# NYXFLOWER/TIP

Measured on AMD Instinct MI355X. Metric: D-D edges aggregated/sec (encoder fwd+bwd), higher is better.
Workload: dtype f32; 1 GPU; TIP-cat full encoder, BioSNAP (645 drugs, 19081 proteins, R=1097), 1xMI355X config; mod=cat, directed_dd_edges=8326508, relations=1097, parallelism=single GPU, launch=hipGraph replay of the captured step, rccl_ranks=0

## Files before the change

tip_amd/csrc/tipk_slab_xb.hip:

```cpp
#include <stdlib.h>
#include "tipk_common.h"

namespace {

struct SxArgs {
    const float* in; int64_t n_slabs, slab_stride; int n_rows;
    const float* row_scale; const float* addend; int relu;
    float* x;
    const float* basis; const float* root; int n_bases, d_out;
    float* xb;
    float* xroot;
};

__global__ __launch_bounds__(1024) void sum_slabs_xb_kernel(SxArgs a) {
    __shared__ float red[1024];
    __shared__ float xs[64];
    constexpr int lanes = 16, epb = 64;
    const int t = threadIdx.x, e = t % epb, j = t / epb;
    const int64_t count = (int64_t)a.n_rows * 32;
    const int64_t i = (int64_t)blockIdx.x * epb + e;
    float s = 0.f;
    if (i < count) {
        const float* p = a.in + i;
        int64_t k = j;
        for (; k + 3 * lanes < a.n_slabs; k += 4 * lanes) {
            const float v0 = p[k * a.slab_stride], v1 = p[(k + lanes) * a.slab_stride];
            const float v2 = p[(k + 2 * lanes) * a.slab_stride], v3 = p[(k + 3 * lanes) * a.slab_stride];
            s += v0; s += v1; s += v2; s += v3;
        }
        for (; k < a.n_slabs; k += lanes) s += p[k * a.slab_stride];
    }
    red[t] = s;
    __syncthreads();
    if (j == 0) {
        float v = 0.f;
        if (i < count) {
            v = red[e];
            for (int q = 1; q < lanes; ++q) v += red[q * epb + e];
            if (a.row_scale) v *= a.row_scale[i / 32];
            if (a.addend) v += a.addend[i];
            if (a.relu) v = fmaxf(v, 0.f);
            a.x[i] = v;
        }
        xs[e] = v;
    }
    __syncthreads();
    const int row0 = (int)blockIdx.x * 2;
    const int n_xb = a.n_bases * a.d_out, n_cols = n_xb + a.d_out;
    for (int n = t; n < n_cols; n += 1024) {
        const bool is_root = n >= n_xb;
        const int b = is_root ? 0 : n / a.d_out, c = is_root ? n - n_xb : n - b * a.d_out;
        const float* w = is_root ? a.root + c : a.basis + (int64_t)b * 32 * a.d_out + c;
        float wv[32];
#pragma unroll
        for (int k = 0; k < 32; ++k) wv[k] = w[k * a.d_out];
        float acc0 = 0.f, acc1 = 0.f;
#pragma unroll
        for (int k = 0; k < 32; ++k) { acc0 = fmaf(xs[k], wv[k], acc0); acc1 = fmaf(xs[32 + k], wv[k], acc1); }
        if (is_root) {
            a.xroot[(int64_t)row0 * a.d_out + c] = acc0;
            if (row0 + 1 < a.n_rows) a.xroot[(int64_t)(row0 + 1) * a.d_out + c] = acc1;
        } else {
            a.xb[((int64_t)row0 * a.n_bases + b) * 32 + c] = acc0;
            if (row0 + 1 < a.n_rows) a.xb[((int64_t)(row0 + 1) * a.n_bases + b) * 32 + c] = acc1;
        }
    }
}

}

extern "C" int tipk_sum_slabs_xb(const float* slabs, int64_t n_slabs, int64_t slab_stride, int64_t n_rows, int d_in,
                                 const float* row_scale, const float* addend, int relu, float* x,
                                 const float* basis, const float* root, int n_bases, int d_out, float* xb, float* xroot,
                                 tipk_stream_t stream) {
    if (d_in != 32 || d_out < 1 || d_out > 32 || n_bases < 1) return TIPK_EUNSUPPORTED;
    if (!slabs || !x || !basis || !root || !xb || !xroot || n_slabs < 1 || n_rows < 1 || slab_stride < n_rows * 32) return TIPK_EINVAL;
    const int64_t blocks = tipk_ceil_div(n_rows, 2);
    if (blocks > 0x7fffffffLL) return TIPK_EUNSUPPORTED;
    SxArgs a;
    a.in = slabs; a.n_slabs = n_slabs; a.slab_stride = slab_stride; a.n_rows = (int)n_rows;
    a.row_scale = row_scale; a.addend = addend; a.relu = relu; a.x = x;
    a.basis = basis; a.root = root; a.n_bases = n_bases; a.d_out = d_out; a.xb = xb; a.xroot = xroot;
    hipLaunchKernelGGL(sum_slabs_xb_kernel, dim3((unsigned)blocks), dim3(1024), 0, (hipStream_t)stream, a);
    TIPK_RETURN_LAUNCH();
}
```

tip_amd/csrc/tipk_slabs.h:

```cpp
#pragma once
#include "tipk_common.h"

namespace {

struct SlabArgs {
    const float* in; int64_t n_slabs, slab_stride, count; float alpha; int accumulate;
    const float* row_scale; int64_t cols; const float* addend; int relu; const float* gate; float* out;
    int lanes;
};
constexpr int SLAB_VEC4 = 1, SLAB_VEC16 = 2;
constexpr int SLAB_RED_FLOATS = 4096;

__device__ __forceinline__ void slab_sum_body(const SlabArgs& a, int block, float* red) {
    const int first = 0;
    const float* __restrict__ in = a.in;
    if (a.lanes == SLAB_VEC16) {
        const int e4 = threadIdx.x & 63, j = threadIdx.x >> 6;
        const int64_t i = (int64_t)(block - first) * 256 + e4 * 4;
        float4 s = make_float4(0.f, 0.f, 0.f, 0.f);
        if (i < a.count) {
            const float4* p = reinterpret_cast<const float4*>(in + i);
            const int64_t st4 = a.slab_stride / 4;
            int64_t k = j;
            for (; k + 48 < a.n_slabs; k += 64) {
                const float4 v0 = p[k * st4], v1 = p[(k + 16) * st4], v2 = p[(k + 32) * st4], v3 = p[(k + 48) * st4];
                s.x += v0.x; s.y += v0.y; s.z += v0.z; s.w += v0.w;
                s.x += v1.x; s.y += v1.y; s.z += v1.z; s.w += v1.w;
                s.x += v2.x; s.y += v2.y; s.z += v2.z; s.w += v2.w;
                s.x += v3.x; s.y += v3.y; s.z += v3.z; s.w += v3.w;
            }
            if (k < a.n_slabs) {
                float4 v[3];
#pragma unroll
                for (int u = 0; u < 3; ++u) v[u] = p[(k + 16 * u < a.n_slabs ? k + 16 * u : k) * st4];
#pragma unroll
                for (int u = 0; u < 3; ++u)
                    if (k + 16 * u < a.n_slabs) { s.x += v[u].x; s.y += v[u].y; s.z += v[u].z; s.w += v[u].w; }
            }
        }
        *reinterpret_cast<float4*>(red + j * 256 + e4 * 4) = s;
        __syncthreads();
        const int e = threadIdx.x;
        const int64_t o = (int64_t)(block - first) * 256 + e;
        if (e < 256 && o < a.count) {
            float t = red[e];
#pragma unroll
            for (int q = 1; q < 16; ++q) t += red[q * 256 + e];
            t *= a.alpha;
            if (a.row_scale) t *= a.row_scale[o / a.cols];
            if (a.addend) t += a.addend[o];
            if (a.accumulate) t += a.out[o];
            if (a.relu) t = fmaxf(t, 0.f);
            if (a.gate && !(a.gate[o] > 0.f)) t = 0.f;
            a.out[o] = t;
        }
        return;
    }
    if (a.lanes == SLAB_VEC4) {
        const int64_t i = ((int64_t)(block - first) * 1024 + threadIdx.x) * 4;
        if (i >= a.count) return;
        const float4* p = reinterpret_cast<const float4*>(in + i);
        const int64_t st4 = a.slab_stride / 4;
        float4 s[4];
#pragma unroll
        for (int j = 0; j < 4; ++j) s[j] = make_float4(0.f, 0.f, 0.f, 0.f);
        int64_t k = 0;
        for (; k + 8 <= a.n_slabs; k += 8) {
            float4 v[8];
#pragma unroll
            for (int u = 0; u < 8; ++u) v[u] = p[(k + u) * st4];
#pragma unroll
            for (int u = 0; u < 8; ++u) { s[u & 3].x += v[u].x; s[u & 3].y += v[u].y; s[u & 3].z += v[u].z; s[u & 3].w += v[u].w; }
        }
        {
            float4 v[8];
#pragma unroll
            for (int u = 0; u < 8; ++u) {
                const int64_t kc = k + u < a.n_slabs ? k + u : (a.n_slabs > 0 ? a.n_slabs - 1 : 0);
                v[u] = a.n_slabs > 0 ? p[kc * st4] : make_float4(0.f, 0.f, 0.f, 0.f);
            }
#pragma unroll
            for (int u = 0; u < 8; ++u)
                if (k + u < a.n_slabs) { s[u & 3].x += v[u].x; s[u & 3].y += v[u].y; s[u & 3].z += v[u].z; s[u & 3].w += v[u].w; }
        }
        float r[4] = {((s[0].x + s[1].x) + s[2].x) + s[3].x, ((s[0].y + s[1].y) + s[2].y) + s[3].y,
                      ((s[0].z + s[1].z) + s[2].z) + s[3].z, ((s[0].w + s[1].w) + s[2].w) + s[3].w};
        const float rs = a.row_scale ? a.row_scale[i / a.cols] : 1.f;
        float4 ad = make_float4(0.f, 0.f, 0.f, 0.f), ac = ad, gt = make_float4(1.f, 1.f, 1.f, 1.f);
        if (a.addend) ad = *reinterpret_cast<const float4*>(a.addend + i);
        if (a.accumulate) ac = *reinterpret_cast<const float4*>(a.out + i);
        if (a.gate) gt = *reinterpret_cast<const float4*>(a.gate + i);
        const float adv[4] = {ad.x, ad.y, ad.z, ad.w}, acv[4] = {ac.x, ac.y, ac.z, ac.w}, gtv[4] = {gt.x, gt.y, gt.z, gt.w};
#pragma unroll
        for (int c = 0; c < 4; ++c) {
            float t = r[c] * a.alpha;
            if (a.row_scale) t *= rs;
            if (a.addend) t += adv[c];
            if (a.accumulate) t += acv[c];
            if (a.relu) t = fmaxf(t, 0.f);
            if (a.gate && !(gtv[c] > 0.f)) t = 0.f;
            r[c] = t;
        }
        *reinterpret_cast<float4*>(a.out + i) = make_float4(r[0], r[1], r[2], r[3]);
        return;
    }
    const int lanes = a.lanes, epb = 1024 / lanes;
    const int e = threadIdx.x % epb, j = threadIdx.x / epb;
    const int64_t i = (int64_t)(block - first) * epb + e;
    float s = 0.f;
    if (i < a.count) {
        const float* p = in + i;
        int64_t k = j;
        for (; k + 3 * lanes < a.n_slabs; k += 4 * lanes) {
            const float v0 = p[k * a.slab_stride], v1 = p[(k + lanes) * a.slab_stride];
            const float v2 = p[(k + 2 * lanes) * a.slab_stride], v3 = p[(k + 3 * lanes) * a.slab_stride];
            s += v0; s += v1; s += v2; s += v3;
        }
        for (; k < a.n_slabs; k += lanes) s += p[k * a.slab_stride];
    }
    red[threadIdx.x] = s;
    __syncthreads();
    if (j == 0 && i < a.count) {
        s = red[e];
        for (int q = 1; q < lanes; ++q) s += red[q * epb + e];
        s *= a.alpha;
        if (a.row_scale) s *= a.row_scale[i / a.cols];
        if (a.addend) s += a.addend[i];
        if (a.accumulate) s += a.out[i];
        if (a.relu) s = fmaxf(s, 0.f);
        if (a.gate && !(a.gate[i] > 0.f)) s = 0.f;
        a.out[i] = s;
    }
}

inline int64_t fill_slab_args(const tipk_slab_sum_desc& d, SlabArgs& a, int* rc) {
    *rc = TIPK_OK;
    if (d.n_slabs < 0 || d.count < 0 || (d.row_scale && d.cols <= 0)) { *rc = TIPK_EINVAL; return 0; }
    if (d.count == 0) return 0;
    if (!d.out || (d.n_slabs > 0 && !d.in)) { *rc = TIPK_EINVAL; return 0; }
    a.in = d.in; a.n_slabs = d.n_slabs; a.slab_stride = d.slab_stride; a.count = d.count; a.alpha = d.alpha;
    a.accumulate = d.accumulate; a.row_scale = d.row_scale; a.cols = d.cols; a.addend = d.addend; a.relu = d.relu;
    a.gate = d.gate; a.out = d.out;
    a.lanes = (d.n_slabs >= 32 && tipk_ceil_div(d.count, 64) < 2048) ? 16 : 4;
    const auto al16 = [](const void* q) { return (reinterpret_cast<uintptr_t>(q) & 15) == 0; };
    const bool vec = d.count % 4 == 0 && d.slab_stride % 4 == 0 && al16(d.in) && al16(d.out) && al16(d.addend) && al16(d.gate) &&
                     (!d.row_scale || d.cols % 4 == 0);
    if (a.lanes == 4 && vec && d.count >= 4096) a.lanes = SLAB_VEC4;
    else if (a.lanes == 16 && vec) a.lanes = SLAB_VEC16;
    if (a.lanes == SLAB_VEC4) return tipk_ceil_div(d.count, 4096);
    if (a.lanes == SLAB_VEC16) return tipk_ceil_div(d.count, 256);
    return tipk_ceil_div(d.count, 1024 / a.lanes);
}

}
```

Before: 42.75 billion edges/s.

## Process eight rows per block in fused slab-sum and basis projection kernel

The fused slab-sum plus basis/root projection kernel now handles 8 rows per block on a float4-vectorized path instead of 2 rows with scalar loads. Each thread's 32 weights are reused across 8 rows, and the weight loads are issued while the slab loads are still in flight. Slab loads for small slab counts are batched, and epilogue operands are fetched early. The cost is more registers and fewer blocks, which may lower occupancy, plus extra template and debug paths.

```diff
diff --git a/tip_amd/csrc/tipk_slab_xb.hip b/tip_amd/csrc/tipk_slab_xb.hip
--- a/tip_amd/csrc/tipk_slab_xb.hip
+++ b/tip_amd/csrc/tipk_slab_xb.hip
@@ -1,68 +1,63 @@
 #include <stdlib.h>
 #include "tipk_common.h"
+#include "tipk_slabs.h"
 
 namespace {
 
 struct SxArgs {
-    const float* in; int64_t n_slabs, slab_stride; int n_rows;
-    const float* row_scale; const float* addend; int relu;
-    float* x;
+    SlabArgs s;
+    int n_rows;
     const float* basis; const float* root; int n_bases, d_out;
     float* xb;
     float* xroot;
 };
 
+template <int ROWS, bool WEARLY>
 __global__ __launch_bounds__(1024) void sum_slabs_xb_kernel(SxArgs a) {
-    __shared__ float red[1024];
-    __shared__ float xs[64];
-    constexpr int lanes = 16, epb = 64;
-    const int t = threadIdx.x, e = t % epb, j = t / epb;
-    const int64_t count = (int64_t)a.n_rows * 32;
-    const int64_t i = (int64_t)blockIdx.x * epb + e;
-    float s = 0.f;
-    if (i < count) {
-        const float* p = a.in + i;
-        int64_t k = j;
-        for (; k + 3 * lanes < a.n_slabs; k += 4 * lanes) {
-            const float v0 = p[k * a.slab_stride], v1 = p[(k + lanes) * a.slab_stride];
-            const float v2 = p[(k + 2 * lanes) * a.slab_stride], v3 = p[(k + 3 * lanes) * a.slab_stride];
-            s += v0; s += v1; s += v2; s += v3;
-        }
-        for (; k < a.n_slabs; k += lanes) s += p[k * a.slab_stride];
-    }
-    red[t] = s;
-    __syncthreads();
-    if (j == 0) {
-        float v = 0.f;
-        if (i < count) {
-            v = red[e];
-            for (int q = 1; q < lanes; ++q) v += red[q * epb + e];
-            if (a.row_scale) v *= a.row_scale[i / 32];
-            if (a.addend) v += a.addend[i];
-            if (a.relu) v = fmaxf(v, 0.f);
-            a.x[i] = v;
-        }
-        xs[e] = v;
-    }
-    __syncthreads();
-    const int row0 = (int)blockIdx.x * 2;
+    __shared__ __attribute__((aligned(16))) float red[ROWS == 8 ? SLAB_RED_FLOATS : 1024];
+    __shared__ __attribute__((aligned(16))) float xs[ROWS * 32];
+    const int t = threadIdx.x;
     const int n_xb = a.n_bases * a.d_out, n_cols = n_xb + a.d_out;
-    for (int n = t; n < n_cols; n += 1024) {
+    float wv[32];
+    auto load_weights = [&](int n) __attribute__((always_inline)) {
         const bool is_root = n >= n_xb;
         const int b = is_root ? 0 : n / a.d_out, c = is_root ? n - n_xb : n - b * a.d_out;
         const float* w = is_root ? a.root + c : a.basis + (int64_t)b * 32 * a.d_out + c;
-        float wv[32];
 #pragma unroll
         for (int k = 0; k < 32; ++k) wv[k] = w[k * a.d_out];
-        float acc0 = 0.f, acc1 = 0.f;
+    };
+    SlabArgs s = a.s;
+    s.lanes = ROWS == 8 ? SLAB_VEC16 : 16;
+    slab_sum_body<true>(s, (int)blockIdx.x, red, xs, [&]() __attribute__((always_inline)) {
+        if (WEARLY && t < n_cols) load_weights(t);
+    });
+    __syncthreads();
+    const int row0 = (int)blockIdx.x * ROWS;
+    for (int n = t; n < n_cols; n += 1024) {
+        if (!WEARLY || n != t) load_weights(n);
+        asm volatile("" ::: "memory");
+        const bool is_root = n >= n_xb;
+        const int b = is_root ? 0 : n / a.d_out, c = is_root ? n - n_xb : n - b * a.d_out;
+        float acc[ROWS];
 #pragma unroll
-        for (int k = 0; k < 32; ++k) { acc0 = fmaf(xs[k], wv[k], acc0); acc1 = fmaf(xs[32 + k], wv[k], acc1); }
-        if (is_root) {
-            a.xroot[(int64_t)row0 * a.d_out + c] = acc0;
-            if (row0 + 1 < a.n_rows) a.xroot[(int64_t)(row0 + 1) * a.d_out + c] = acc1;
-        } else {
-            a.xb[((int64_t)row0 * a.n_bases + b) * 32 + c] = acc0;
-            if (row0 + 1 < a.n_rows) a.xb[((int64_t)(row0 + 1) * a.n_bases + b) * 32 + c] = acc1;
+        for (int r = 0; r < ROWS; ++r) acc[r] = 0.f;
+#pragma unroll
+        for (int k = 0; k < 32; k += 4) {
+            __builtin_amdgcn_sched_barrier(0);
+#pragma unroll
+            for (int r = 0; r < ROWS; ++r) {
+                const float4 xv = *reinterpret_cast<const float4*>(xs + r * 32 + k);
+                acc[r] = fmaf(xv.x, wv[k], acc[r]); acc[r] = fmaf(xv.y, wv[k + 1], acc[r]);
+                acc[r] = fmaf(xv.z, wv[k + 2], acc[r]); acc[r] = fmaf(xv.w, wv[k + 3], acc[r]);
+            }
+        }
+#pragma unroll
+        for (int r = 0; r < ROWS; ++r) asm volatile("" : "+v"(acc[r]));
+#pragma unroll
+        for (int r = 0; r < ROWS; ++r) {
+            if (row0 + r >= a.n_rows) break;
+            if (is_root) a.xroot[(int64_t)(row0 + r) * a.d_out + c] = acc[r];
+            else a.xb[((int64_t)(row0 + r) * a.n_bases + b) * 32 + c] = acc[r];
         }
     }
 }
@@ -75,12 +70,29 @@
                                  tipk_stream_t stream) {
     if (d_in != 32 || d_out < 1 || d_out > 32 || n_bases < 1) return TIPK_EUNSUPPORTED;
     if (!slabs || !x || !basis || !root || !xb || !xroot || n_slabs < 1 || n_rows < 1 || slab_stride < n_rows * 32) return TIPK_EINVAL;
-    const int64_t blocks = tipk_ceil_div(n_rows, 2);
-    if (blocks > 0x7fffffffLL) return TIPK_EUNSUPPORTED;
     SxArgs a;
-    a.in = slabs; a.n_slabs = n_slabs; a.slab_stride = slab_stride; a.n_rows = (int)n_rows;
-    a.row_scale = row_scale; a.addend = addend; a.relu = relu; a.x = x;
+    a.s.in = slabs; a.s.n_slabs = n_slabs; a.s.slab_stride = slab_stride; a.s.count = n_rows * 32; a.s.alpha = 1.f;
+    a.s.accumulate = 0; a.s.row_scale = row_scale; a.s.cols = 32; a.s.addend = addend; a.s.relu = relu; a.s.gate = nullptr;
+    a.s.out = x;
+    a.n_rows = (int)n_rows;
     a.basis = basis; a.root = root; a.n_bases = n_bases; a.d_out = d_out; a.xb = xb; a.xroot = xroot;
-    hipLaunchKernelGGL(sum_slabs_xb_kernel, dim3((unsigned)blocks), dim3(1024), 0, (hipStream_t)stream, a);
+    const int dbg = tipk_option(TIPK_OPT_DP_DEBUG);
+    (void)dbg;
+    const auto al16 = [](const void* q) { return (reinterpret_cast<uintptr_t>(q) & 15) == 0; };
+    const bool vec = slab_stride % 4 == 0 && al16(slabs) && al16(x) && al16(addend) && !TIPK_DBG(dbg & 4096);
+    a.s.lanes = vec ? SLAB_VEC16 : 16;
+    const int64_t blocks = tipk_ceil_div(n_rows, vec ? 8 : 2);
+    if (blocks > 0x7fffffffLL || n_rows > 0x7fffffffLL / 32) return TIPK_EUNSUPPORTED;
+    const dim3 grid((unsigned)blocks), block(1024);
+    hipStream_t st = (hipStream_t)stream;
+#ifdef TIPK_DEBUG
+    if (dbg & 8192) {
+        if (vec) hipLaunchKernelGGL((sum_slabs_xb_kernel<8, false>), grid, block, 0, st, a);
+        else hipLaunchKernelGGL((sum_slabs_xb_kernel<2, false>), grid, block, 0, st, a);
+        TIPK_RETURN_LAUNCH();
+    }
+#endif
+    if (vec) hipLaunchKernelGGL((sum_slabs_xb_kernel<8, true>), grid, block, 0, st, a);
+    else hipLaunchKernelGGL((sum_slabs_xb_kernel<2, true>), grid, block, 0, st, a);
     TIPK_RETURN_LAUNCH();
 }
diff --git a/tip_amd/csrc/tipk_slabs.h b/tip_amd/csrc/tipk_slabs.h
--- a/tip_amd/csrc/tipk_slabs.h
+++ b/tip_amd/csrc/tipk_slabs.h
@@ -11,9 +11,116 @@
 constexpr int SLAB_VEC4 = 1, SLAB_VEC16 = 2;
 constexpr int SLAB_RED_FLOATS = 4096;
 
-__device__ __forceinline__ void slab_sum_body(const SlabArgs& a, int block, float* red) {
+constexpr int SLAB_BATCH = 6;
+struct SlabNoHook { __device__ __forceinline__ void operator()() const {} };
+
+struct SlabEpilogue { float rs, ad, ac; bool open; };
+__device__ __forceinline__ SlabEpilogue slab_epilogue_loads(const SlabArgs& a, int64_t o, bool fin) {
+    SlabEpilogue q = {1.f, 0.f, 0.f, true};
+    if (fin) {
+        if (a.row_scale) q.rs = a.row_scale[o / a.cols];
+        if (a.addend) q.ad = a.addend[o];
+        if (a.accumulate) q.ac = a.out[o];
+        if (a.gate) q.open = a.gate[o] > 0.f;
+    }
+    return q;
+}
+__device__ __forceinline__ float slab_epilogue(const SlabArgs& a, float t, const SlabEpilogue& q) {
+    t = __fmul_rn(t, a.alpha);
+    if (a.row_scale) t = __fmul_rn(t, q.rs);
+    if (a.addend) t = __fadd_rn(t, q.ad);
+    if (a.accumulate) t = __fadd_rn(t, q.ac);
+    if (a.relu) t = fmaxf(t, 0.f);
+    if (a.gate && !q.open) t = 0.f;
+    return t;
+}
+
+template <bool CHAIN = false, class Hook = SlabNoHook>
+__device__ __forceinline__ void slab_sum_body(const SlabArgs& a, int block, float* red, float* keep = nullptr, Hook after_issue = Hook()) {
     const int first = 0;
     const float* __restrict__ in = a.in;
+    if (CHAIN && (a.lanes == SLAB_VEC16 || a.lanes == 16)) {
+        const bool vec = a.lanes == SLAB_VEC16;
+        const int epb = vec ? 256 : 64, e = threadIdx.x, j = threadIdx.x >> 6;
+        const int64_t o = (int64_t)block * epb + e;
+        const bool fin = e < epb && o < a.count;
+        const bool batch = a.n_slabs > 0 && a.n_slabs <= 16 * SLAB_BATCH;
+        SlabEpilogue q;
+        if (vec) {
+            const int e4 = threadIdx.x & 63;
+            const int64_t i = (int64_t)block * 256 + e4 * 4;
+            const bool live = i < a.count;
+            const float4* p = reinterpret_cast<const float4*>(in + (live ? i : 0));
+            const int64_t st4 = a.slab_stride / 4;
+            float4 s = make_float4(0.f, 0.f, 0.f, 0.f);
+            if (batch) {
+                float4 v[SLAB_BATCH];
+#pragma unroll
+                for (int u = 0; u < SLAB_BATCH; ++u) v[u] = p[(j + 16 * u < a.n_slabs ? j + 16 * u : 0) * st4];
+                q = slab_epilogue_loads(a, o, fin);
+                after_issue();
+#pragma unroll
+                for (int u = 0; u < SLAB_BATCH; ++u)
+                    if (live && j + 16 * u < a.n_slabs) { s.x += v[u].x; s.y += v[u].y; s.z += v[u].z; s.w += v[u].w; }
+            } else {
+                q = slab_epilogue_loads(a, o, fin);
+                after_issue();
+                if (live) {
+                    int64_t k = j;
+                    for (; k + 48 < a.n_slabs; k += 64) {
+                        const float4 v0 = p[k * st4], v1 = p[(k + 16) * st4], v2 = p[(k + 32) * st4], v3 = p[(k + 48) * st4];
+                        s.x += v0.x; s.y += v0.y; s.z += v0.z; s.w += v0.w;
+                        s.x += v1.x; s.y += v1.y; s.z += v1.z; s.w += v1.w;
+                        s.x += v2.x; s.y += v2.y; s.z += v2.z; s.w += v2.w;
+                        s.x += v3.x; s.y += v3.y; s.z += v3.z; s.w += v3.w;
+                    }
+                    for (; k < a.n_slabs; k += 16) { const float4 v0 = p[k * st4]; s.x += v0.x; s.y += v0.y; s.z += v0.z; s.w += v0.w; }
+                }
+            }
+            *reinterpret_cast<float4*>(red + j * 256 + e4 * 4) = s;
+        } else {
+            const int64_t i = (int64_t)block * 64 + (threadIdx.x & 63);
+            const bool live = i < a.count;
+            const float* p = in + (live ? i : 0);
+            float s = 0.f;
+            if (batch) {
+                float v[SLAB_BATCH];
+#pragma unroll
+                for (int u = 0; u < SLAB_BATCH; ++u) v[u] = p[(j + 16 * u < a.n_slabs ? j + 16 * u : 0) * a.slab_stride];
+                q = slab_epilogue_loads(a, o, fin);
+                after_issue();
+#pragma unroll
+                for (int u = 0; u < SLAB_BATCH; ++u)
+                    if (live && j + 16 * u < a.n_slabs) s += v[u];
+            } else {
+                q = slab_epilogue_loads(a, o, fin);
+                after_issue();
+                if (live) {
+                    int64_t k = j;
+                    for (; k + 48 < a.n_slabs; k += 64) {
+                        const float v0 = p[k * a.slab_stride], v1 = p[(k + 16) * a.slab_stride];
+                        const float v2 = p[(k + 32) * a.slab_stride], v3 = p[(k + 48) * a.slab_stride];
+                        s += v0; s += v1; s += v2; s += v3;
+                    }
+                    for (; k < a.n_slabs; k += 16) s += p[k * a.slab_stride];
+                }
+            }
+            red[threadIdx.x] = s;
+        }
+        __syncthreads();
+        if (e < epb) {
+            float t = 0.f;
+            if (fin) {
+                t = red[e];
+#pragma unroll
+                for (int r = 1; r < 16; ++r) t += red[r * epb + e];
+                t = slab_epilogue(a, t, q);
+                a.out[o] = t;
+            }
+            if (keep) keep[e] = t;
+        }
+        return;
+    }
     if (a.lanes == SLAB_VEC16) {
         const int e4 = threadIdx.x & 63, j = threadIdx.x >> 6;
         const int64_t i = (int64_t)(block - first) * 256 + e4 * 4;
```

Result: no change. 42.84 billion edges/s, median of 2 (+0.2%).
